# k-sheridan/mantis

Hardware: AMD Instinct MI355X
Metric: poses/sec + p50 per-frame latency, 1280x720 4-cam batch (higher is better)
Workload: dtype f64; 1 GPU; config3: 4-cam 1280x720 rig, shared map, full mantis3 path per camera + joint rig Gauss-Newton; cams_per_rig=4, contexts_per_gpu=6, landmarks=720, parallelism=rig-data-parallel x1

## Files before the change

### include/mantis.h

```cpp
#ifndef MANTIS_H
#define MANTIS_H
#include <stddef.h>
#include <stdint.h>

#ifdef __cplusplus
extern "C" {
#endif

#define MANTIS_ABI_VERSION 5

typedef enum mantis_status {
  MANTIS_OK = 0,
  MANTIS_ERR_ARG = 1,
  MANTIS_ERR_DEVICE = 2,
  MANTIS_ERR_OOM = 3,
  MANTIS_ERR_CAPACITY = 4,
  MANTIS_ERR_STATE = 5,
  MANTIS_ERR_COMM = 6
} mantis_status;

typedef enum mantis_reason {
  MANTIS_PUBLISHED = 0,
  MANTIS_NO_QUADS = 1,
  MANTIS_NO_HYPS = 2,
// ... 90 lines not shown
                                   mantis_result* out, mantis_cam_result* cam_out);

mantis_status mantis_process_rig_sharded(void* ctx, const mantis_image* local_cams, int32_t n_rigs, int32_t n_local,
                                         const int32_t* cam_index, int32_t cams_per_rig, mantis_result* out,
                                         mantis_cam_result* cam_out);

mantis_status mantis_shard_gauss_offsets(void* ctx, const int32_t* pairs, int32_t npairs, int32_t n_global,
                                         const int32_t* gidx, int32_t n_local, int32_t per_frame, int32_t* offsets,
                                         int32_t* total);

typedef struct mantis_rig_gn_info {
  double T_init[16];
  double T_final[16];
  double cost0, cost;
  int32_t valid, iterations, n_obs, n_obs_local;
} mantis_rig_gn_info;
mantis_status mantis_get_rig_gn(void* ctx, int32_t rig, mantis_rig_gn_info* info, double* obs, int32_t cap);

mantis_status mantis_get_rig_weights(void* ctx, int32_t rig, double* weights, double* c2w, double* sums,
                                     int32_t* chosen);
mantis_status mantis_get_rig_weights_info(void* ctx, int32_t* n_rigs, int32_t* cams_per_rig);

mantis_status mantis_markov_init(void* ctx, int32_t n_filters, const double* w2c_R);
mantis_status mantis_markov_sense(void* ctx, const double* w2c_R, const int32_t* active);
mantis_status mantis_markov_convolve(void* ctx, const double* dtheta, const double* dt, const int32_t* active);
mantis_status mantis_markov_weight(void* ctx, int32_t filter, const double* w2c_R, int32_t n, double* error);
mantis_status mantis_markov_get(void* ctx, double* planes, double* yaw, int32_t* argmax);

mantis_status mantis_canny(void* ctx, const mantis_image* img, uint8_t* canny_out);
mantis_status mantis_hysteresis(void* ctx, const uint8_t* cls, int32_t width, int32_t height, uint8_t* edges_out);
mantis_status mantis_masks(void* ctx, const mantis_image* img, uint8_t* det_out, uint8_t* mask_out);
mantis_status mantis_detect_quads(void* ctx, const mantis_image* img, int32_t* corners, int32_t max_quads,
                                  int32_t* n_quads);
mantis_status mantis_score_hypotheses(void* ctx, const mantis_image* img, const uint8_t* mask, const double* c2w,
                                      int32_t n, int32_t fast, double* err, int32_t* nproj);
mantis_status mantis_rpp_batch(void* ctx, const double* img_pts, const double* obj_pts, int32_t n, double* R,
                               double* t, double* errs, int32_t* rpp_status);
mantis_status mantis_rpp_solve(void* ctx, const double* img_pts, const double* obj_pts, int32_t n_points,
                               int32_t n, double* R, double* t, double* errs, int32_t* rpp_status,
                               int32_t* iterations);

mantis_status mantis_quad_gn(void* ctx, const double* img_pts, const double* obj_pts, int32_t n, double* R,
                             double* t, int32_t iterations, int32_t* steps, double* costs);

mantis_status mantis_score_argmin(void* ctx, const mantis_image* img, const uint8_t* mask, const double* c2w,
                                  int32_t n, int64_t index_base, int32_t use_comm, double* best_err,
                                  int64_t* best_idx);
mantis_status mantis_score_argmin_dev(void* ctx, const mantis_image* img, const uint8_t* mask_dev,
                                      const double* c2w_dev, int32_t n, int64_t index_base, int32_t use_comm,
                                      double* best_err, int64_t* best_idx);
mantis_status mantis_argmin_pick(const double* pairs, int32_t nranks, double* best_err, int64_t* best_idx);

mantis_status mantis_score_argmin_batch(void* ctx, const mantis_image* imgs, int32_t n_frames,
                                        const uint8_t* const* masks_dev, const double* const* c2w_dev,
                                        const int32_t* n_hyps, const int64_t* index_base, int32_t use_comm,
                                        double* best_err, int64_t* best_idx);

mantis_status mantis_gn_accumulate(void* ctx, const double* T_w_b, const double* T_base_cam, int32_t n_cams,
                                   const double* obs, int32_t n_obs, double* acc28);
mantis_status mantis_gn_solve(const double* acc28, double lambda, double* T_w_b, double* delta6);

mantis_status mantis_comm_unique_id(void* id128);
mantis_status mantis_comm_init(void* ctx, const void* id128, int32_t nranks, int32_t rank);
mantis_status mantis_comm_info(void* ctx, int32_t* nranks, int32_t* rank);
mantis_status mantis_gn_allreduce(void* ctx, double* acc28);

// ... 391 lines not shown
```

### mantis_amd/__init__.py

```python
import ctypes as C
import os

import numpy as np

ROOT = os.path.dirname(os.path.dirname(os.path.abspath(__file__)))
LIB_PATH = os.environ.get("MANTIS_AMD_LIB") or os.path.join(os.path.dirname(os.path.abspath(__file__)),
                                                             "libmantis_amd.so")

MANTIS_OK = 0
REASONS = {0: "published", 1: "no_quads", 2: "no_hyps", 3: "yaw_ambiguous", 4: "no_yaw"}


class MantisConfig(C.Structure):
    _fields_ = [("struct_size", C.c_int32), ("device", C.c_int32), ("max_cams", C.c_int32),
                ("max_width", C.c_int32), ("max_height", C.c_int32), ("rng_seed", C.c_uint64),
                ("canny_low", C.c_int32), ("polygon_epsilon", C.c_int32),
                ("search_radius_multiplier", C.c_double), ("grid_spacing", C.c_double),
                ("particles", C.c_int32), ("iterations", C.c_int32), ("gn_enable", C.c_int32),
                ("gn_iterations", C.c_int32), ("max_quads", C.c_int32), ("max_contour_points", C.c_int32),
                ("quad_gn_iterations", C.c_int32), ("rig_weighting", C.c_int32)]


class MantisImage(C.Structure):
    _fields_ = [("width", C.c_int32), ("height", C.c_int32), ("step_bytes", C.c_int32), ("mem_kind", C.c_int32),
# ... 191 lines not shown
        ("quads", (C.c_int32 * 8) * 256), ("test_pts", (C.c_double * 8) * 256),
        ("n_gen", C.c_int32), ("n_hyps", C.c_int32),
        ("hyp_c2w", (C.c_double * 12) * 1024), ("hyp_err", C.c_double * 1024), ("hyp_n", C.c_int32 * 1024),
        ("best1_c2w", C.c_double * 12), ("best1_err", C.c_double),
        ("pf_c2w", C.c_double * 12), ("pf_err", C.c_double), ("pf_iter_err", C.c_double * 11),
        ("shift_err", C.c_double * 81), ("top20_err", C.c_double * 20), ("yaw_err", C.c_double * 4),
        ("yaw_best", C.c_int32), ("min_yaw_diff", C.c_double), ("pub_c2w", C.c_double * 12),
        ("pub_error", C.c_double), ("position", C.c_double * 3), ("orientation_xyzw", C.c_double * 4),
        ("covariance", C.c_double * 36), ("rng_state_after", C.c_uint64), ("n_scored", C.c_int32),
    ]


_lib = None

_SIGS = {
    "mantis_abi_version": (C.c_int32, []),
    "mantis_default_config": (None, [C.POINTER(MantisConfig)]),
    "mantis_create": (C.c_int, [C.POINTER(MantisConfig), C.POINTER(C.c_void_p)]),
    "mantis_destroy": (C.c_int, [C.c_void_p]),
    "mantis_last_error": (C.c_char_p, [C.c_void_p]),
    "mantis_set_map": (C.c_int, [C.c_void_p, C.c_void_p, C.c_int32, C.c_void_p, C.c_int32, C.c_void_p, C.c_int32]),
    "mantis_parse_coordinates": (C.c_int32, [C.c_char_p, C.c_void_p, C.c_int32]),
    "mantis_rng_get": (C.c_int, [C.c_void_p, C.POINTER(C.c_uint64)]),
    "mantis_rng_set": (C.c_int, [C.c_void_p, C.c_uint64]),
    "mantis_process": (C.c_int, [C.c_void_p, C.POINTER(MantisImage), C.c_int32, C.POINTER(MantisMotion),
                                 C.POINTER(MantisResult), C.POINTER(MantisCamResult)]),
    "mantis_process_batch": (C.c_int, [C.c_void_p, C.POINTER(MantisImage), C.c_int32, C.c_int32,
                                       C.POINTER(MantisResult), C.POINTER(MantisCamResult)]),
    "mantis_canny": (C.c_int, [C.c_void_p, C.POINTER(MantisImage), C.c_void_p]),
    "mantis_hysteresis": (C.c_int, [C.c_void_p, C.c_void_p, C.c_int32, C.c_int32, C.c_void_p]),
    "mantis_masks": (C.c_int, [C.c_void_p, C.POINTER(MantisImage), C.c_void_p, C.c_void_p]),
    "mantis_detect_quads": (C.c_int, [C.c_void_p, C.POINTER(MantisImage), C.c_void_p, C.c_int32,
                                      C.POINTER(C.c_int32)]),
    "mantis_score_hypotheses": (C.c_int, [C.c_void_p, C.POINTER(MantisImage), C.c_void_p, C.c_void_p, C.c_int32,
                                          C.c_int32, C.c_void_p, C.c_void_p]),
    "mantis_rpp_batch": (C.c_int, [C.c_void_p, C.c_void_p, C.c_void_p, C.c_int32, C.c_void_p, C.c_void_p,
                                   C.c_void_p, C.c_void_p]),
    "mantis_small_batch_frames": (C.c_int32, [C.c_void_p]),
    "mantis_rpp_solve": (C.c_int, [C.c_void_p, C.c_void_p, C.c_void_p, C.c_int32, C.c_int32, C.c_void_p,
                                   C.c_void_p, C.c_void_p, C.c_void_p, C.c_void_p]),
    "mantis_quad_gn": (C.c_int, [C.c_void_p, C.c_void_p, C.c_void_p, C.c_int32, C.c_void_p, C.c_void_p, C.c_int32,
                                 C.c_void_p, C.c_void_p]),
    "mantis_get_rig_weights": (C.c_int, [C.c_void_p, C.c_int32, C.c_void_p, C.c_void_p, C.c_void_p,
                                         C.POINTER(C.c_int32)]),
    "mantis_markov_init": (C.c_int, [C.c_void_p, C.c_int32, C.c_void_p]),
    "mantis_markov_sense": (C.c_int, [C.c_void_p, C.c_void_p, C.c_void_p]),
    "mantis_markov_convolve": (C.c_int, [C.c_void_p, C.c_void_p, C.c_void_p, C.c_void_p]),
    "mantis_markov_weight": (C.c_int, [C.c_void_p, C.c_int32, C.c_void_p, C.c_int32, C.c_void_p]),
    "mantis_markov_get": (C.c_int, [C.c_void_p, C.c_void_p, C.c_void_p, C.c_void_p]),
    "mantis_set_prior_pose": (C.c_int, [C.c_void_p, C.c_void_p]),
    "mantis_get_prior_pose": (C.c_int, [C.c_void_p, C.c_void_p, C.POINTER(C.c_int32)]),
    "mantis_synth_render": (C.c_int, [C.c_void_p, C.POINTER(SynthCamC), C.c_int32, C.c_void_p, C.c_void_p]),
    "mantis_device_alloc": (C.c_int, [C.c_void_p, C.c_size_t, C.POINTER(C.c_void_p)]),
    "mantis_device_free": (C.c_int, [C.c_void_p, C.c_void_p]),
    "mantis_memcpy_h2d": (C.c_int, [C.c_void_p, C.c_void_p, C.c_void_p, C.c_size_t]),
    "mantis_memcpy_d2h": (C.c_int, [C.c_void_p, C.c_void_p, C.c_void_p, C.c_size_t]),
    "mantis_synchronize": (C.c_int, [C.c_void_p]),
    "mantis_kernel_times": (C.c_int32, [C.c_void_p, C.POINTER(C.c_char_p), C.POINTER(C.c_float), C.c_int32]),
    "mantis_set_profiling": (C.c_int, [C.c_void_p, C.c_int32]),
    "mantis_frame_debug_size": (C.c_size_t, []),
    "mantis_get_frame_debug": (C.c_int, [C.c_void_p, C.c_int32, C.c_void_p, C.c_size_t]),
    "mantis_get_contours": (C.c_int, [C.c_void_p, C.c_int32, C.c_void_p, C.c_void_p, C.c_int32, C.c_void_p, C.c_int32,
                                      C.c_void_p]),
    "mantis_frame_counters": (C.c_int32, [C.c_void_p, C.c_int32, C.c_void_p, C.c_int32]),
    "mantis_gn_accumulate": (C.c_int, [C.c_void_p, C.c_void_p, C.c_void_p, C.c_int32, C.c_void_p, C.c_int32,
                                       C.c_void_p]),
# ... 910 lines not shown
        return out[:k]

    def frame_debug(self, i):
        d = FrameDebug()
        assert C.sizeof(d) == lib().mantis_frame_debug_size(), "FrameDebug layout mismatch"
        self._chk(lib().mantis_get_frame_debug(self.h, i, C.byref(d), C.sizeof(d)), "get_frame_debug")
        return d

    def canny(self, img):
        out = np.zeros((img.height, img.width), np.uint8)
        self._chk(lib().mantis_canny(self.h, C.byref(img), out.ctypes.data), "canny")
        return out

    def hysteresis(self, cls):
        cls = np.ascontiguousarray(cls, np.uint8)
        h, w = cls.shape
        out = np.zeros((h, w), np.uint8)
        self._chk(lib().mantis_hysteresis(self.h, cls.ctypes.data, w, h, out.ctypes.data), "hysteresis")
        return out

    def masks(self, img):
        det = np.zeros((img.height, img.width), np.uint8)
        mask = np.zeros((img.height, img.width), np.uint8)
        self._chk(lib().mantis_masks(self.h, C.byref(img), det.ctypes.data, mask.ctypes.data), "masks")
        return det, mask

    def detect_quads(self, img, max_quads=256):
        corners = np.zeros((max_quads, 8), np.int32)
        n = C.c_int32()
        self._chk(lib().mantis_detect_quads(self.h, C.byref(img), corners.ctypes.data, max_quads, C.byref(n)),
                  "detect_quads")
        return corners[: n.value].copy()

    def score(self, img, c2w, fast=True, mask=None):
        c2w = np.ascontiguousarray(c2w, np.float64).reshape(-1, 12)
        n = len(c2w)
        err = np.zeros(n)
        npj = np.zeros(n, np.int32)
        mptr = None
        if mask is not None:
            mask = np.ascontiguousarray(mask, np.uint8)
            mptr = mask.ctypes.data
        self._chk(lib().mantis_score_hypotheses(self.h, C.byref(img), mptr, c2w.ctypes.data, n, int(fast),
                                                err.ctypes.data, npj.ctypes.data), "score_hypotheses")
        return err, npj

    def comm_init(self, rank, world, dist=None):
        uid = (C.c_uint8 * 128)()
        if rank == 0:
            self._chk(lib().mantis_comm_unique_id(uid), "comm_unique_id")
        if dist is not None and world > 1:
            box = [bytes(uid)]
            dist.broadcast_object_list(box, src=0)
            C.memmove(uid, box[0], 128)
        self._chk(lib().mantis_comm_init(self.h, uid, world, rank), "comm_init")

    def score_argmin(self, img, c2w, index_base=0, use_comm=False, mask=None):
        c2w = np.ascontiguousarray(c2w, np.float64).reshape(-1, 12)
        e = C.c_double()
        i = C.c_int64()
        mk = None if mask is None else np.ascontiguousarray(mask, np.uint8)
        self._chk(lib().mantis_score_argmin(self.h, C.byref(img), None if mk is None else mk.ctypes.data,
                                            c2w.ctypes.data, len(c2w), index_base, int(use_comm), C.byref(e),
                                            C.byref(i)), "score_argmin")
        return e.value, i.value

# ... 177 lines not shown
```

### mantis_amd/csrc/api.hip

```cpp
#include <hip/hip_runtime.h>
#ifndef MK_FC_THREADS
#define MK_FC_THREADS 256
#endif

#include <algorithm>
#include <atomic>
#include <cfloat>
#include <chrono>
#include <cmath>
#include <cstdio>
#include <cstdlib>
#include <cstring>
#include <mutex>
#include <sstream>
#include <string>
#include <thread>
#include <vector>

#include <rccl/rccl.h>

#include "hostbuf.h"
#include "kernels.hip"

namespace mk {
// ... 555 lines not shown
mantis_status run_hyst_ccl(Ctx* c, int n, int W, int H, bool edge_bytes) {
  const size_t P = c->plane, B = c->bstride;
  c->hyst_epoch = c->hyst_epoch >= 255 ? 4 : c->hyst_epoch + 1;
  if (c->hyst_epoch == 4) HIP_OK(hipMemsetAsync(c->d_strong, 0, c->fstride * (size_t)c->F, c->s));
  HystRuns hr{(uint32_t*)c->d_lroot.get(), c->d_lab, c->d_strong, c->d_rowb, c->lstride / 2, P, c->fstride, c->rstride, P / 2,
              HB_ROWS * ((W + 1) / 2), c->d_st, c->hyst_epoch};
  HIP_OK(hipMemset2DAsync(c->d_rowb + H + 1, c->rstride * sizeof(int32_t), 0, 2 * sizeof(int32_t), n, c->s));
  const int WWb = bits::words(W);
  k_hyst_band<<<dim3((H + HB_ROWS - 1) / HB_ROWS, n), HB_THREADS, 3 * sizeof(uint32_t) * HB_ROWS * WWb, c->s>>>(
      c->d_b1, c->d_b2, B, hr, c->d_eb, W, H);
  mark(c, "hysteresis/k_hyst_band");
  const int nseam = (H - 1) / HB_ROWS;
  if (nseam > 0) k_hyst_seam<<<dim3((nseam + 3) / 4, n), 256, 0, c->s>>>(hr, H);
  mark(c, "hysteresis/k_hyst_seam");
  k_hyst_mark<<<dim3(8, n), 256, 0, c->s>>>(hr, H);
  mark(c, "hysteresis/k_hyst_mark");
  k_hyst_fix<<<dim3(8, n), 256, 0, c->s>>>(hr, c->d_eb, B, W, H);
  if (edge_bytes) k_bits_to_bytes<<<blocks_for((size_t)W * H), 256, 0, c->s>>>(c->d_eb, c->d_edge, W, H, 0);
  mark(c, "hysteresis/k_hyst_fix");
  HIP_OK(hipGetLastError());
  return MANTIS_OK;
}

mantis_status run_contours(Ctx* c, int n, int W, int H) {
  const size_t P = c->plane;
  const int Wp = W + 2, Hp = H + 2;
  dim3 grow((Hp + 4 * RUN_RPW - 1) / (4 * RUN_RPW), n);
  uint16_t* rx = c->d_lroot;
  if (!c->runs_done) {
    k_run_count<<<grow, 256, 0, c->s>>>(c->d_dbits, c->dstride, c->d_rowb, c->rstride, Wp, Hp);
    k_run_scan<<<n, 256, 0, c->s>>>(c->d_rowb, c->rstride, c->d_st, Hp);
    k_run_emit<<<grow, 256, 0, c->s>>>(c->d_dbits, c->dstride, c->d_rowb, c->rstride, rx, c->d_lab, P, Wp, Hp);
  }
  k_run_band<<<dim3((Hp + RB_ROWS - 1) / RB_ROWS, n), RB_THREADS, 0, c->s>>>(c->d_rowb, c->rstride, rx, c->d_lab, P, Wp, Hp);
  const int seams = (Hp - 1) / RB_ROWS;
  if (seams > 0)
    k_run_seam<<<dim3((seams + 3) / 4, n), 256, 0, c->s>>>(c->d_rowb, c->rstride, rx, c->d_lab, P, Wp, Hp);
  k_run_border<<<grow, 256, 0, c->s>>>(c->d_rowb, c->rstride, rx, c->d_lab, P, c->d_borders, c->d_st, Wp, Hp,
                                       kMaxBorders);
  mark(c, "components");
  const size_t tb_lds = (size_t)dbits_wpw(Wp) * Hp * sizeof(uint32_t);
  k_seg_plan<<<n, 256, 0, c->s>>>(c->d_dbits, c->dstride, c->d_rowb, c->rstride, rx, c->d_lab, P, c->d_borders,
                                  c->d_st, c->d_scratch, c->pool_cap, Wp, Hp, kMaxBorders, c->seg_m);
  if (trace_on_lds(c, n, Wp, Hp)) {
    k_trace_borders_lds<<<n, 1024, tb_lds, c->s>>>(c->d_dbits, c->dstride, c->d_borders, c->d_st, c->d_scratch,
                                                   c->pool_cap, Wp, Hp, kMaxBorders, c->d_rowb, c->rstride, rx, P);
  } else {
    const int wpw = dbits_wpw(Wp);
    k_tile_bits<<<dim3((Hp + 31) / 32, n), 256, kTbRows * wpw * sizeof(uint32_t), c->s>>>(
        c->d_dbits, c->dstride, c->d_tbits, c->tstride, wpw, Wp, Hp);
    k_trace_borders<<<n, 64 * MK_TB_WAVES, 0, c->s>>>(c->d_tbits, c->tstride, c->d_borders, c->d_st, c->d_scratch, c->pool_cap, Wp,
                                        kMaxBorders, c->d_rowb, c->rstride, rx, P);
  }
  k_seg_chain<<<n, 256, 0, c->s>>>(c->d_st, c->d_bcount, c->d_scratch, c->pool_cap, kMaxBorders);
  mark(c, "border_trace");
  k_frame_contours<<<n, n <= c->fc_small_frames ? 1024 : MK_FC_THREADS, 0, c->s>>>(c->d_dbits, c->dstride, c->d_borders, c->d_st, c->d_bcount, c->d_boff,
                                         c->d_pool, c->d_scratch, c->pool_cap, c->d_quads, c->d_dbg, c->d_frames, Wp,
                                         Hp, P, kMaxBorders, (double)c->cfg.polygon_epsilon,
                                         c->cfg.search_radius_multiplier, c->d_rowb, c->rstride, rx);
  mark(c, "contours_quads");
  HIP_OK(hipGetLastError());
  return MANTIS_OK;
}

std::atomic<int> g_live_ctx[64];

unsigned objpose_blocks(const Ctx* c, size_t expected_jobs) {
  size_t b = (expected_jobs + 127) / 128;
  const int live = std::max(1, g_live_ctx[c->cfg.device & 63].load());
  const size_t cap = c->rpp_blocks > 0 ? (size_t)c->rpp_blocks : (size_t)std::max(64, 3 * c->n_cu / (2 * live));
  return (unsigned)std::max<size_t>(1, std::min(b, cap));
}
// ... 1147 lines not shown
    HIP_OK(hipMemcpyAsync(mask_out, c->d_mask, (size_t)W * H, hipMemcpyDeviceToHost, c->s));
  }
  HIP_OK(hipStreamSynchronize(c->s));
  for (size_t i = 0; det_out && i < (size_t)W * H; i++) det_out[i] = det_out[i] ? 255 : 0;
  for (size_t i = 0; mask_out && i < (size_t)W * H; i++) mask_out[i] = mask_out[i] ? 255 : 0;
  return MANTIS_OK;
}

mantis_status mantis_detect_quads(void* ctx, const mantis_image* img, int32_t* corners, int32_t max_quads,
                                  int32_t* n_quads) {
  Ctx* c = (Ctx*)ctx;
  if (c) bind_device(c);
  if (!c || !img || !n_quads) return MANTIS_ERR_ARG;
  int W, H;
  mantis_status st = stage_frames(c, img, 1, W, H);
  if (st != MANTIS_OK) return st;
  c->frame_rng.clear();
  if ((st = run_image_stages(c, 1, W, H)) != MANTIS_OK) return st;
  if ((st = run_contours(c, 1, W, H)) != MANTIS_OK) return st;
  HIP_OK(hipMemcpyAsync(c->h_st, c->d_st, sizeof(FrameState), hipMemcpyDeviceToHost, c->s));
  HIP_OK(hipStreamSynchronize(c->s));
  if (c->h_st[0].overflow) { c->err = "detect_quads: workspace capacity exceeded"; return MANTIS_ERR_CAPACITY; }
  int nq = c->h_st[0].n_quads;
  *n_quads = nq;
  if (corners && max_quads > 0) {
    std::vector<QuadRec> q(nq);
    HIP_OK(hipMemcpy(q.data(), c->d_quads, sizeof(QuadRec) * nq, hipMemcpyDeviceToHost));
    for (int i = 0; i < nq && i < max_quads; i++)
      for (int k = 0; k < 8; k++) corners[8 * i + k] = q[i].c[k];
  }
  return MANTIS_OK;
}

mantis_status mantis_score_hypotheses(void* ctx, const mantis_image* img, const uint8_t* mask, const double* c2w,
                                      int32_t n, int32_t fast, double* err, int32_t* nproj) {
  Ctx* c = (Ctx*)ctx;
  if (c) bind_device(c);
  if (!c || !img || !c2w || n <= 0 || !err || !nproj) return MANTIS_ERR_ARG;
  if (!c->d_lm) { c->err = "map not set"; return MANTIS_ERR_STATE; }
  int W, H;
  mantis_status st = stage_frames(c, img, 1, W, H);
  if (st != MANTIS_OK) return st;
  double* d_c2w = nullptr;
  double* d_err = nullptr;
  int32_t* d_np = nullptr;
  DevScratch ds(c);
  if (ds.get(&d_c2w, (size_t)12 * n) || ds.get(&d_err, (size_t)n) || ds.get(&d_np, (size_t)n)) return MANTIS_ERR_OOM;
  const uint8_t* d_mask = nullptr;
  if (mask) {
    HIP_OK(hipMemcpyAsync(c->d_mask, mask, (size_t)W * H, hipMemcpyHostToDevice, c->s));
    d_mask = c->d_mask;
  }
  HIP_OK(hipMemcpyAsync(d_c2w, c2w, sizeof(double) * 12 * n, hipMemcpyHostToDevice, c->s));
  Landmarks L = lmk_of(c);
  mark(c, "start");
  k_score_api<<<(n + kApiHyps - 1) / kApiHyps, 64 * kApiHyps, 0, c->s>>>(c->d_frames, d_mask, L, d_c2w, n, fast, d_err, d_np);
  mark(c, "score_api");
  HIP_OK(hipGetLastError());
  HIP_OK(hipMemcpyAsync(err, d_err, sizeof(double) * n, hipMemcpyDeviceToHost, c->s));
  HIP_OK(hipMemcpyAsync(nproj, d_np, sizeof(int32_t) * n, hipMemcpyDeviceToHost, c->s));
  HIP_OK(hipStreamSynchronize(c->s));
  finish_profile(c);
  return MANTIS_OK;
}

mantis_status mantis_quad_gn(void* ctx, const double* img_pts, const double* obj_pts, int32_t n, double* R,
// ... 202 lines not shown
```

### mantis_amd/csrc/kernels.hip

```cpp
#include <hip/hip_runtime.h>

#include <cfloat>
#include <cstdint>
#include <type_traits>

#include "mk_bits.h"
#include "mk_contour.h"
#include "mk_gn.h"
#include "mk_math.h"
#include "mk_rpp.h"
#include "mk_shard.h"
#include "mk_sort.h"
#include "mk_track.h"
#include "mk_types.h"
#include "synth.h"

namespace mk {

#ifndef MK_DPP_SCAN
#define MK_DPP_SCAN 1
#endif
__device__ inline int wave_incl_scan(int v, int lane) {
#if MK_DPP_SCAN
  (void)lane;
// ... 1707 lines not shown
        T &= T - 1;
        X[o] = (uint16_t)(32 * w + b);
        L[o] = o;
        o++;
      }
      base += __builtin_amdgcn_readlane(inc, 63);
    }
  }
}

__device__ inline int run_at(const uint16_t* x, int n, int v) {
  int lo = 0, hi = n - 1;
  while (lo < hi) {
    const int mid = (lo + hi + 1) >> 1;
    if ((int)x[mid] <= v) lo = mid;
    else hi = mid - 1;
  }
  return lo;
}

template <class UF>
__device__ inline void run_row_union(const uint16_t* X, int bp, int np, int by, int ny, int Wp, int lane,
                                     const UF& uni) {
  const uint16_t* Xp = X + bp;
  for (int j = lane; j < ny; j += 64) {
    const int fg = j & 1;
    const int a = X[by + j], b = (j + 1 < ny ? (int)X[by + j + 1] : Wp) - 1;
    const int lo = a - fg, hi = b + fg;
    for (int k = run_at(Xp, np, lo); k < np && (int)Xp[k] <= hi; k++)
      if ((k & 1) == fg) uni(by + j, bp + k);
  }
}

#ifndef MK_RB_ROWS
#define MK_RB_ROWS 32
#endif
constexpr int RB_ROWS = MK_RB_ROWS, RB_CAP = 128 * MK_RB_ROWS;
#ifndef MK_RB_THREADS
#define MK_RB_THREADS 512
#endif
constexpr int RB_THREADS = MK_RB_THREADS, RB_WAVES = RB_THREADS / 64;
__global__ __launch_bounds__(RB_THREADS) void k_run_band(const int32_t* __restrict__ rowb, size_t rstride,
                                                  const uint16_t* __restrict__ rx, int32_t* lab, size_t plane, int Wp,
                                                  int Hp) {
  __shared__ int32_t Ll[RB_CAP];
  __shared__ uint16_t Xl[RB_CAP];
  __shared__ int32_t rbl[RB_ROWS + 1];
  const int f = blockIdx.y, t = threadIdx.x, lane = t & 63, wave = t >> 6;
  const int y0 = blockIdx.x * RB_ROWS;
  if (y0 >= Hp) return;
  const int y1 = min(y0 + RB_ROWS, Hp);
  const int32_t* r = rowb + (size_t)f * rstride;
  const uint16_t* X = rx + (size_t)f * plane;
  int32_t* L = lab + (size_t)f * plane;
  const int g0 = r[y0], n = r[y1] - g0;
  if (n > RB_CAP) {
    const auto uni = [L](int a, int b) { uf_union_c(L, a, b); };
    for (int y = y0 + 1 + wave; y < y1; y += RB_WAVES) run_row_union(X, r[y - 1], r[y] - r[y - 1], r[y], r[y + 1] - r[y], Wp, lane, uni);
    return;
  }
  for (int i = t; i <= y1 - y0; i += RB_THREADS) rbl[i] = r[y0 + i] - g0;
  for (int i = t; i < n; i += RB_THREADS) {
    Xl[i] = X[g0 + i];
    Ll[i] = i;
  }
  __syncthreads();
  int* Li = Ll;
  const auto uni = [Li](int a, int b) { lds_union(Li, a, b); };
  for (int y = y0 + 1 + wave; y < y1; y += RB_WAVES) {
    const int q = y - y0;
    run_row_union(Xl, rbl[q - 1], rbl[q] - rbl[q - 1], rbl[q], rbl[q + 1] - rbl[q], Wp, lane, uni);
  }
  __syncthreads();
  for (int i = t; i < n; i += RB_THREADS) L[g0 + i] = g0 + lds_find(Ll, i);
}

__global__ __launch_bounds__(256) void k_run_seam(const int32_t* __restrict__ rowb, size_t rstride,
                                                  const uint16_t* __restrict__ rx, int32_t* lab, size_t plane, int Wp,
                                                  int Hp) {
  const int f = blockIdx.y;
  const int y = (blockIdx.x * 4 + (threadIdx.x >> 6) + 1) * RB_ROWS, lane = threadIdx.x & 63;
  if (y >= Hp) return;
  const int32_t* r = rowb + (size_t)f * rstride;
  int32_t* L = lab + (size_t)f * plane;
  const auto uni = [L](int a, int b) { uf_union_c(L, a, b); };
  run_row_union(rx + (size_t)f * plane, r[y - 1], r[y] - r[y - 1], r[y], r[y + 1] - r[y], Wp, lane, uni);
}

__device__ inline int run_at_row(const int32_t* rowb, int Hp, int id) {
  int lo = 0, hi = Hp - 1;
  while (lo < hi) {
    const int mid = (lo + hi + 1) >> 1;
    if (rowb[mid] <= id) lo = mid;
    else hi = mid - 1;
  }
  return lo;
}

__global__ __launch_bounds__(256) void k_run_border(const int32_t* __restrict__ rowb, size_t rstride,
                                                    const uint16_t* __restrict__ rx, int32_t* lab, size_t plane,
                                                    Border* __restrict__ borders, FrameState* st, int Wp, int Hp,
                                                    int cap) {
  const int f = blockIdx.y, lane = threadIdx.x & 63;
  const int ya = (blockIdx.x * 4 + (threadIdx.x >> 6)) * RUN_RPW, yb = min(ya + RUN_RPW, Hp);
  if (ya >= Hp) return;
  const int32_t* r = rowb + (size_t)f * rstride;
  const uint16_t* X = rx + (size_t)f * plane;
  int32_t* L = lab + (size_t)f * plane;
  const int nrow = yb - ya;
  const int rbq = lane <= nrow ? r[ya + lane] : 0x7fffffff;
  const int g0 = __builtin_amdgcn_readlane(rbq, 0), g1 = __builtin_amdgcn_readlane(rbq, nrow);
  const int nruns = r[Hp];
  const uint64_t below = (1ull << lane) - 1;
  for (int id = g0 + lane; __ballot(id < g1); id += 64) {
    const bool live = id < g1;
    int y = ya, by = g0;
#pragma unroll
    for (int k = 1; k < RUN_RPW; k++) {
      const int bk = __builtin_amdgcn_readlane(rbq, k);
      if (k < nrow && bk <= id) { y = ya + k; by = bk; }
    }
    const int j = id - by;
    const bool root = live && id != 0 && L[id] == id;
    Border b;
    if (root) {
      const int key = y * Wp + X[id];
      b.key = key;
      if (j & 1) {
        b.start = key; b.hole = 0; b.parent = key;
      } else {
        const int pr = uf_find_c(L, id - 1);
        b.start = key - 1; b.hole = 1; b.parent = -(pr + 1);
      }
    }
    const uint64_t m = __ballot(root);
    if (!m) continue;
    const int leader = __ffsll((unsigned long long)m) - 1;
    int base = 0;
    if (lane == leader) base = atomicAdd(&st[f].n_borders, __popcll(m));
    base = __builtin_amdgcn_readlane(base, leader);
    if (!root) continue;
    const int idx = base + __popcll(m & below);
    if (idx < cap) {
      borders[(size_t)f * cap + idx] = b;
      if (2 * (size_t)nruns <= plane) L[nruns + id] = idx;
    } else {
      atomicOr(&st[f].overflow, 1);
    }
  }
}

__device__ inline int fdx(int s) { return (int)((0x901Au >> (2 * s)) & 3u) - 1; }
__device__ inline int fdy(int s) { return (int)((0xA901u >> (2 * s)) & 3u) - 1; }

__device__ inline void build_next_lut(uint8_t* lut, int tid, int nthreads) {
  for (int e = tid; e < 512 * 8; e += nthreads) {
    const uint32_t p9 = (uint32_t)e >> 3;
    const int s = e & 7;
    const uint32_t m = nb8_from_rows(p9 & 7u, (p9 >> 3) & 7u, (p9 >> 6) & 7u);
    const uint32_t r = ((m | (m << 8)) >> (s + 1)) & 0xffu;
    lut[e] = r ? (uint8_t)((s + 1 + __builtin_ctz(r)) & 7) : (uint8_t)8;
  }
}

constexpr int kChunk = 16;
#ifndef MK_CHUNK_BUF
#define MK_CHUNK_BUF 2
#endif
struct ChunkEmit {
  int32_t* chunks;
  int32_t* owner;
  int32_t* ordv;
  int32_t* ccount;
  int32_t* counter;
  int max_chunks, border, cur, k, nch;
  bool ovf;
  int n_pts = 0;
#if MK_CHUNK_BUF
#if MK_CHUNK_BUF == 2
  uint32_t bp[8];
  __device__ uint32_t pk(int j) const { return bp[j]; }
// ... 320 lines not shown
      return false;
    }
  }
  w.first = 0;
  if (s != w.prev_s) {
    em(x - 1, y - 1);
    w.n++;
    w.prev_s = s;
  }
  const uint32_t np = w.pos + wdelta(s);
  if (np == w.spos && w.pos == w.p1) {
    nx = -1;
    return false;
  }
  w.pos = np;
  w.s = (s + 4) & 7;
  w.steps++;
  return true;
}

struct BitsRows {
  const uint32_t* b;
  int wpw;
  __device__ uint32_t row3(int x, int y) const {
    const uint32_t* p = b + (size_t)y * wpw + ((x - 1) >> 5);
    const uint64_t v = ((uint64_t)p[1] << 32) | p[0];
    return (uint32_t)(v >> ((x - 1) & 31)) & 7u;
  }
  __device__ uint32_t operator()(int x, int y) const { return nb8_from_rows(row3(x, y - 1), row3(x, y), row3(x, y + 1)); }
};
__global__ __launch_bounds__(256) void k_seg_plan(const uint32_t* __restrict__ dbits, size_t dstride,
                                                  const int32_t* __restrict__ rowb, size_t rstride,
                                                  const uint16_t* __restrict__ rx, int32_t* lab, size_t plane,
                                                  const Border* __restrict__ borders, FrameState* st,
                                                  int32_t* __restrict__ scratch, int pool_cap, int Wp, int Hp,
                                                  int border_cap, int M) {
  __shared__ int32_t rb[kSegRows + 1];
  __shared__ int32_t wsum[4];
  const int f = blockIdx.x, t = threadIdx.x, lane = t & 63, wave = t >> 6;
  const int32_t* r = rowb + (size_t)f * rstride;
  const uint16_t* X = rx + (size_t)f * plane;
  int32_t* L = lab + (size_t)f * plane;
  const int nruns = r[Hp];
  const int32_t* bidx = L + nruns;
  int nb = st[f].n_borders;
  if (nb > border_cap) nb = border_cap;
  SegTab T = seg_tab(scratch + 4 * (size_t)f * pool_cap, pool_cap);
  if (nb > T.cap) {
    if (t == 0) atomicOr(&st[f].overflow, 2);
    nb = T.cap;
  }
  const Border* bs = borders + (size_t)f * border_cap;
  const int nsr = M > 0 ? (Hp - 2) / M : 0;
  bool split = M > 0 && nsr > 0 && nsr <= kSegRows && 2 * (size_t)nruns <= plane;
  static_assert(kSegRows <= 512, "two passes of 256 sampled rows");
  int carry = 0;
  for (int pass = 0; pass < 2; pass++) {
    int v = 0;
    const int k = pass * 256 + t;
    if (split && k < nsr) {
      const int y = (k + 1) * M;
      v = 2 * ((r[y + 1] - r[y] - 1) >> 1);
    }
    const int inc = wave_incl_scan(v, lane);
    if (lane == 63) wsum[wave] = inc;
    __syncthreads();
    int o = carry;
    for (int q = 0; q < wave; q++) o += wsum[q];
    if (k < kSegRows) rb[k] = o + inc - v;
    carry += wsum[0] + wsum[1] + wsum[2] + wsum[3];
    __syncthreads();
  }
  int NC = split ? carry : 0;
  if (NC + nb > T.cap) {
    split = false;
    NC = 0;
  }
  if (t == 0) {
    st[f].seg_nc = NC;
    st[f].seg_m = split ? M : 0;
  }
  for (int k = t; k < nsr && split; k += 256) T.rowbase[k] = rb[k];
  const BitsRows nbh{dbits + (size_t)f * dstride, dbits_wpw(Wp)};
  if (split) {
    for (int k = 0; k < nsr; k++) {
// ... 178 lines not shown
      continue;
    }
    if (nidle == 64) {
      if (exhausted) break;
      continue;
    }
    int nx = -1;
    if (act && !walk_step(nbh.b, nbh.G, next_lut, em, w, M, r, X, T.rowbase, nx)) {
      act = false;
      finish(nx);
    }
  }
  if (lane == 0) atomicMax(&st[f].trace_ticks, (int32_t)(wall_clock64() - t_start));
}

extern __shared__ uint32_t tb_lds[];
struct BitsNBLds {
  int wpw;
  __device__ uint32_t row3(int x, int y) const {
    const int o = y * wpw + ((x - 1) >> 5);
    const uint64_t v = ((uint64_t)tb_lds[o + 1] << 32) | tb_lds[o];
    return (uint32_t)(v >> ((x - 1) & 31)) & 7u;
  }
  __device__ uint32_t operator()(int x, int y) const { return nb8_from_rows(row3(x, y - 1), row3(x, y), row3(x, y + 1)); }
};
template <class NB, class EM>
__device__ inline int walk_segment_lds(const NB& nb, const uint8_t* lut, EM& em, const Border& b, int Wp,
                                       uint32_t pos, int sd, int M, const int32_t* r, const uint16_t* X,
                                       const int32_t* rowbase, int& steps) {
  Walk w;
  if (sd == kSegStart) {
    if (!walk_start(nb, b.start % Wp, b.start / Wp, b.hole != 0, em, w)) {
      steps = 0;
      return -1;
    }
    w.first = 0;
  } else {
    seg_begin(nb, b, Wp, pos, sd, w);
  }
  for (;;) {
    const int x = (int)(w.pos & 0xffffu), y = (int)(w.pos >> 16);
    const uint32_t p9 = nb.row3(x, y - 1) | (nb.row3(x, y) << 3) | (nb.row3(x, y + 1) << 6);
    const int s = lut[(p9 << 3) | w.s];
    if (M > 0 && !w.first && y % M == 0) {
      const bool west = arc_has(w.s, s, 4);
      if (west || arc_has(w.s, s, 0)) {
        steps = w.steps;
        em.n_pts = w.n;
        return seg_id_at(x, y, west ? 0 : 1, M, r, X, rowbase);
      }
    }
    w.first = 0;
    if (s != w.prev_s) {
      em(x - 1, y - 1);
      w.n++;
      w.prev_s = s;
    }
    const uint32_t np = w.pos + wdelta(s);
    if (np == w.spos && w.pos == w.p1) break;
    w.pos = np;
    w.s = (s + 4) & 7;
    w.steps++;
  }
  steps = w.steps;
  em.n_pts = w.n;
  return -1;
// ... 2331 lines not shown
```

### mantis_amd/csrc/mk_types.h

```cpp
#pragma once
#include <cstdint>

#include "../../include/mantis.h"
#include "mk_math.h"
#include "mk_screen.h"

namespace mk {

constexpr int kLandmarksMax = 2048;
constexpr int kGaussPerFrame = 3000;
constexpr int kMaxQuads = 256;
constexpr int kMaxHyps = 4 * kMaxQuads;
constexpr int kMaxBorders = 8192;

struct FrameDesc {
  const uint8_t* bgr;
  int32_t w, h;
  Cam cam;
  ScreenCam scam;
};

struct Border {
  int32_t key;
  int32_t start;
// ... 46 lines not shown
  double top20_err[20];
  double yaw_err[4];
  int32_t yaw_best;
  double min_yaw_diff;
  double pub_c2w[12];
  double pub_error;
  double position[3];
  double orientation_xyzw[4];
  double covariance[36];
  uint64_t rng_state_after;
  int32_t n_scored;
};


struct FrameState {
  int32_t n_borders;
  int32_t n_points;
  int32_t n_raw_quads;
  int32_t n_quads;
  int32_t n_gen;
  int32_t n_hyps;
  int32_t reaches_pf;
  int32_t gauss_offset;
  int32_t overflow;
  int32_t n_runs;
  int32_t ticks[6];
  int32_t rpp_iters[2];
  int32_t trace_steps_max;
  int32_t n_chunks;
  int32_t trace_steps_sum;
  int32_t trace_ticks;
  int32_t seg_nc;
  int32_t seg_m;
};

struct GnCam {
  double R_cb[9];
  double t_cb[3];
};
struct RigGnIO {
  double Twb[16];
  double T0[16];
  double cost0, cost;
  int32_t valid, iterations, n_obs, done;
  int32_t n_obs_local, pad[3];
};
constexpr int kGnSlot = 32;

constexpr int kYawBins = 360;

struct MarkovOp {
  int32_t kind;
  int32_t bin;
  int32_t off;
  int32_t pad;
  double den;
  double E[181];
};


}
```

Measured before the change: 30580 rig poses/s.

## Fuse border emission into band union and segment planning via root candidate lists

Removes the separate k_run_border kernel, which scanned every run to find union-find roots. k_run_band now records root candidates, and for oversized bands every run as a candidate, into a per-frame scratch list. k_seg_plan then emits borders from that compact list, falling back to a full scan when the list overflows. This saves a kernel launch and a full pass over runs, but puts border emission on one block per frame and reuses scratch space that seg_plan also uses for its tables. It also adds a debug API for contours on binary planes and fixes n_pts on a failed walk start.

```diff
diff --git a/include/mantis.h b/include/mantis.h
--- a/include/mantis.h
+++ b/include/mantis.h
@@ -146,6 +146,7 @@
 mantis_status mantis_masks(void* ctx, const mantis_image* img, uint8_t* det_out, uint8_t* mask_out);
 mantis_status mantis_detect_quads(void* ctx, const mantis_image* img, int32_t* corners, int32_t max_quads,
                                   int32_t* n_quads);
+mantis_status mantis_contours_of_binary(void* ctx, const uint8_t* planes, int32_t n, int32_t width, int32_t height);
 mantis_status mantis_score_hypotheses(void* ctx, const mantis_image* img, const uint8_t* mask, const double* c2w,
                                       int32_t n, int32_t fast, double* err, int32_t* nproj);
 mantis_status mantis_rpp_batch(void* ctx, const double* img_pts, const double* obj_pts, int32_t n, double* R,
diff --git a/mantis_amd/__init__.py b/mantis_amd/__init__.py
--- a/mantis_amd/__init__.py
+++ b/mantis_amd/__init__.py
@@ -247,6 +247,7 @@
     "mantis_masks": (C.c_int, [C.c_void_p, C.POINTER(MantisImage), C.c_void_p, C.c_void_p]),
     "mantis_detect_quads": (C.c_int, [C.c_void_p, C.POINTER(MantisImage), C.c_void_p, C.c_int32,
                                       C.POINTER(C.c_int32)]),
+    "mantis_contours_of_binary": (C.c_int, [C.c_void_p, C.c_void_p, C.c_int32, C.c_int32, C.c_int32]),
     "mantis_score_hypotheses": (C.c_int, [C.c_void_p, C.POINTER(MantisImage), C.c_void_p, C.c_void_p, C.c_int32,
                                           C.c_int32, C.c_void_p, C.c_void_p]),
     "mantis_rpp_batch": (C.c_int, [C.c_void_p, C.c_void_p, C.c_void_p, C.c_int32, C.c_void_p, C.c_void_p,
@@ -1223,6 +1224,13 @@
                   "detect_quads")
         return corners[: n.value].copy()
 
+    def contours_of_binary(self, planes):
+        planes = np.ascontiguousarray(planes, np.uint8)
+        if planes.ndim == 2:
+            planes = planes[None]
+        n, h, w = planes.shape
+        self._chk(lib().mantis_contours_of_binary(self.h, planes.ctypes.data, n, w, h), "contours_of_binary")
+
     def score(self, img, c2w, fast=True, mask=None):
         c2w = np.ascontiguousarray(c2w, np.float64).reshape(-1, 12)
         n = len(c2w)
diff --git a/mantis_amd/csrc/api.hip b/mantis_amd/csrc/api.hip
--- a/mantis_amd/csrc/api.hip
+++ b/mantis_amd/csrc/api.hip
@@ -611,12 +611,11 @@
     k_run_scan<<<n, 256, 0, c->s>>>(c->d_rowb, c->rstride, c->d_st, Hp);
     k_run_emit<<<grow, 256, 0, c->s>>>(c->d_dbits, c->dstride, c->d_rowb, c->rstride, rx, c->d_lab, P, Wp, Hp);
   }
-  k_run_band<<<dim3((Hp + RB_ROWS - 1) / RB_ROWS, n), RB_THREADS, 0, c->s>>>(c->d_rowb, c->rstride, rx, c->d_lab, P, Wp, Hp);
+  k_run_band<<<dim3((Hp + RB_ROWS - 1) / RB_ROWS, n), RB_THREADS, 0, c->s>>>(c->d_rowb, c->rstride, rx, c->d_lab, P, Wp, Hp,
+                                                                             c->d_st, c->d_scratch, c->pool_cap);
   const int seams = (Hp - 1) / RB_ROWS;
   if (seams > 0)
     k_run_seam<<<dim3((seams + 3) / 4, n), 256, 0, c->s>>>(c->d_rowb, c->rstride, rx, c->d_lab, P, Wp, Hp);
-  k_run_border<<<grow, 256, 0, c->s>>>(c->d_rowb, c->rstride, rx, c->d_lab, P, c->d_borders, c->d_st, Wp, Hp,
-                                       kMaxBorders);
   mark(c, "components");
   const size_t tb_lds = (size_t)dbits_wpw(Wp) * Hp * sizeof(uint32_t);
   k_seg_plan<<<n, 256, 0, c->s>>>(c->d_dbits, c->dstride, c->d_rowb, c->rstride, rx, c->d_lab, P, c->d_borders,
@@ -1830,6 +1829,38 @@
   return MANTIS_OK;
 }
 
+mantis_status mantis_contours_of_binary(void* ctx, const uint8_t* planes, int32_t n, int32_t width, int32_t height) {
+  Ctx* c = (Ctx*)ctx;
+  if (c) bind_device(c);
+  if (!c || !planes) return MANTIS_ERR_ARG;
+  const int W = width, H = height;
+  if (n <= 0 || n > c->F) { c->err = "frame count exceeds max_cams"; return MANTIS_ERR_ARG; }
+  if (W <= 2 || H <= 2 || W > c->Wmax || H > c->Hmax) { c->err = "image size outside [3, max]"; return MANTIS_ERR_ARG; }
+  const int Wp = W + 2, Hp = H + 2, wpw = dbits_wpw(Wp);
+  std::vector<uint32_t> bits((size_t)wpw * Hp);
+  for (int f = 0; f < n; f++) {
+    std::fill(bits.begin(), bits.end(), 0u);
+    const uint8_t* pl = planes + (size_t)f * W * H;
+    for (int y = 0; y < H; y++)
+      for (int x = 0; x < W; x++)
+        if (pl[(size_t)y * W + x]) bits[(size_t)(y + 1) * wpw + ((x + 1) >> 5)] |= 1u << ((x + 1) & 31);
+    HIP_OK(hipMemcpy(c->d_dbits + (size_t)f * c->dstride, bits.data(), sizeof(uint32_t) * bits.size(), hipMemcpyHostToDevice));
+    FrameDesc& fd = c->h_frames[f];
+    std::memset(&fd, 0, sizeof(fd));
+    fd.w = W;
+    fd.h = H;
+    fd.cam.fx = fd.cam.fy = 1.0;
+  }
+  HIP_OK(hipMemcpyAsync(c->d_frames, c->h_frames, sizeof(FrameDesc) * n, hipMemcpyHostToDevice, c->s));
+  c->frame_rng.clear();
+  HIP_OK(hipMemsetAsync(c->d_st, 0, sizeof(FrameState) * n, c->s));
+  c->runs_done = false;
+  if (mantis_status st = run_contours(c, n, W, H); st != MANTIS_OK) return st;
+  HIP_OK(hipMemcpyAsync(c->h_st, c->d_st, sizeof(FrameState) * n, hipMemcpyDeviceToHost, c->s));
+  HIP_OK(hipStreamSynchronize(c->s));
+  return MANTIS_OK;
+}
+
 mantis_status mantis_score_hypotheses(void* ctx, const mantis_image* img, const uint8_t* mask, const double* c2w,
                                       int32_t n, int32_t fast, double* err, int32_t* nproj) {
   Ctx* c = (Ctx*)ctx;
diff --git a/mantis_amd/csrc/kernels.hip b/mantis_amd/csrc/kernels.hip
--- a/mantis_amd/csrc/kernels.hip
+++ b/mantis_amd/csrc/kernels.hip
@@ -1763,6 +1763,13 @@
   }
 }
 
+struct RootCands {
+  int2* e;
+  int cap;
+};
+__device__ inline RootCands root_cands(int32_t* scratch, int f, int pool_cap) {
+  return RootCands{(int2*)(scratch + 4 * (size_t)f * pool_cap), pool_cap};
+}
 #ifndef MK_RB_ROWS
 #define MK_RB_ROWS 32
 #endif
@@ -1773,10 +1780,12 @@
 constexpr int RB_THREADS = MK_RB_THREADS, RB_WAVES = RB_THREADS / 64;
 __global__ __launch_bounds__(RB_THREADS) void k_run_band(const int32_t* __restrict__ rowb, size_t rstride,
                                                   const uint16_t* __restrict__ rx, int32_t* lab, size_t plane, int Wp,
-                                                  int Hp) {
+                                                  int Hp, FrameState* st, int32_t* __restrict__ scratch,
+                                                  int pool_cap) {
   __shared__ int32_t Ll[RB_CAP];
   __shared__ uint16_t Xl[RB_CAP];
   __shared__ int32_t rbl[RB_ROWS + 1];
+  __shared__ int32_t ncand, cbase;
   const int f = blockIdx.y, t = threadIdx.x, lane = t & 63, wave = t >> 6;
   const int y0 = blockIdx.x * RB_ROWS;
   if (y0 >= Hp) return;
@@ -1784,12 +1793,21 @@
   const int32_t* r = rowb + (size_t)f * rstride;
   const uint16_t* X = rx + (size_t)f * plane;
   int32_t* L = lab + (size_t)f * plane;
+  const RootCands C = root_cands(scratch, f, pool_cap);
   const int g0 = r[y0], n = r[y1] - g0;
   if (n > RB_CAP) {
+    if (t == 0) cbase = atomicAdd(&st[f].n_cand, n);
     const auto uni = [L](int a, int b) { uf_union_c(L, a, b); };
     for (int y = y0 + 1 + wave; y < y1; y += RB_WAVES) run_row_union(X, r[y - 1], r[y] - r[y - 1], r[y], r[y + 1] - r[y], Wp, lane, uni);
+    __syncthreads();
+    for (int y = y0 + wave; y < y1; y += RB_WAVES)
+      for (int j = r[y] + lane; j < r[y + 1]; j += 64) {
+        const int pos = cbase + (j - g0);
+        if (pos < C.cap) C.e[pos] = make_int2(j, y);
+      }
     return;
   }
+  if (t == 0) ncand = 0;
   for (int i = t; i <= y1 - y0; i += RB_THREADS) rbl[i] = r[y0 + i] - g0;
   for (int i = t; i < n; i += RB_THREADS) {
     Xl[i] = X[g0 + i];
@@ -1803,7 +1821,35 @@
     run_row_union(Xl, rbl[q - 1], rbl[q] - rbl[q - 1], rbl[q], rbl[q + 1] - rbl[q], Wp, lane, uni);
   }
   __syncthreads();
-  for (int i = t; i < n; i += RB_THREADS) L[g0 + i] = g0 + lds_find(Ll, i);
+  const uint64_t below = (1ull << lane) - 1;
+  for (int i0 = 0; i0 < n; i0 += RB_THREADS) {
+    const int i = i0 + t;
+    bool root = false;
+    if (i < n) {
+      const int rt = lds_find(Ll, i);
+      L[g0 + i] = g0 + rt;
+      root = rt == i && g0 + i != 0;
+    }
+    const uint64_t m = __ballot(root);
+    if (!m) continue;
+    const int leader = __ffsll((unsigned long long)m) - 1;
+    int base = 0;
+    if (lane == leader) base = atomicAdd(&ncand, __popcll(m));
+    base = __builtin_amdgcn_readlane(base, leader);
+    if (root) Xl[base + __popcll(m & below)] = (uint16_t)i;
+  }
+  __syncthreads();
+  const int nc = ncand;
+  if (t == 0) cbase = atomicAdd(&st[f].n_cand, nc);
+  __syncthreads();
+  for (int k = t; k < nc; k += RB_THREADS) {
+    const int i = Xl[k], pos = cbase + k;
+    int q = 0;
+    static_assert(RB_ROWS <= 64, "row search steps 32 .. 1");
+    for (int s = 32; s > 0; s >>= 1)
+      if (q + s < y1 - y0 && rbl[q + s] <= i) q += s;
+    if (pos < C.cap) C.e[pos] = make_int2(g0 + i, y0 + q);
+  }
 }
 
 __global__ __launch_bounds__(256) void k_run_seam(const int32_t* __restrict__ rowb, size_t rstride,
@@ -1828,56 +1874,42 @@
   return lo;
 }
 
-__global__ __launch_bounds__(256) void k_run_border(const int32_t* __restrict__ rowb, size_t rstride,
-                                                    const uint16_t* __restrict__ rx, int32_t* lab, size_t plane,
-                                                    Border* __restrict__ borders, FrameState* st, int Wp, int Hp,
-                                                    int cap) {
-  const int f = blockIdx.y, lane = threadIdx.x & 63;
-  const int ya = (blockIdx.x * 4 + (threadIdx.x >> 6)) * RUN_RPW, yb = min(ya + RUN_RPW, Hp);
-  if (ya >= Hp) return;
-  const int32_t* r = rowb + (size_t)f * rstride;
-  const uint16_t* X = rx + (size_t)f * plane;
-  int32_t* L = lab + (size_t)f * plane;
-  const int nrow = yb - ya;
-  const int rbq = lane <= nrow ? r[ya + lane] : 0x7fffffff;
-  const int g0 = __builtin_amdgcn_readlane(rbq, 0), g1 = __builtin_amdgcn_readlane(rbq, nrow);
-  const int nruns = r[Hp];
-  const uint64_t below = (1ull << lane) - 1;
-  for (int id = g0 + lane; __ballot(id < g1); id += 64) {
-    const bool live = id < g1;
-    int y = ya, by = g0;
-#pragma unroll
-    for (int k = 1; k < RUN_RPW; k++) {
-      const int bk = __builtin_amdgcn_readlane(rbq, k);
-      if (k < nrow && bk <= id) { y = ya + k; by = bk; }
-    }
-    const int j = id - by;
-    const bool root = live && id != 0 && L[id] == id;
-    Border b;
-    if (root) {
-      const int key = y * Wp + X[id];
-      b.key = key;
-      if (j & 1) {
-        b.start = key; b.hole = 0; b.parent = key;
-      } else {
-        const int pr = uf_find_c(L, id - 1);
-        b.start = key - 1; b.hole = 1; b.parent = -(pr + 1);
-      }
-    }
-    const uint64_t m = __ballot(root);
-    if (!m) continue;
-    const int leader = __ffsll((unsigned long long)m) - 1;
-    int base = 0;
-    if (lane == leader) base = atomicAdd(&st[f].n_borders, __popcll(m));
-    base = __builtin_amdgcn_readlane(base, leader);
-    if (!root) continue;
-    const int idx = base + __popcll(m & below);
-    if (idx < cap) {
-      borders[(size_t)f * cap + idx] = b;
-      if (2 * (size_t)nruns <= plane) L[nruns + id] = idx;
+struct RunPlanes {
+  const int32_t* r;
+  const uint16_t* X;
+  int32_t* L;
+  int nruns;
+  bool map_fits;
+};
+__device__ inline void run_border_trip(const RunPlanes& P, bool live, int id, int y, Border* borders, int cap,
+                                       int32_t* nbord, int32_t* overflow, int Wp, int lane) {
+  int32_t* L = P.L;
+  const bool root = live && id != 0 && L[id] == id;
+  Border b;
+  if (root) {
+    const int j = id - P.r[y];
+    const int key = y * Wp + P.X[id];
+    b.key = key;
+    if (j & 1) {
+      b.start = key; b.hole = 0; b.parent = key;
     } else {
-      atomicOr(&st[f].overflow, 1);
-    }
+      const int pr = uf_find_c(L, id - 1);
+      b.start = key - 1; b.hole = 1; b.parent = -(pr + 1);
+    }
+  }
+  const uint64_t m = __ballot(root);
+  if (!m) return;
+  const int leader = __ffsll((unsigned long long)m) - 1;
+  int base = 0;
+  if (lane == leader) base = atomicAdd(nbord, __popcll(m));
+  base = __builtin_amdgcn_readlane(base, leader);
+  if (!root) return;
+  const int idx = base + __popcll(m & ((1ull << lane) - 1));
+  if (idx < cap) {
+    borders[idx] = b;
+    if (P.map_fits) L[P.nruns + id] = idx;
+  } else {
+    atomicOr(overflow, 1);
   }
 }
 
@@ -2264,25 +2296,49 @@
 __global__ __launch_bounds__(256) void k_seg_plan(const uint32_t* __restrict__ dbits, size_t dstride,
                                                   const int32_t* __restrict__ rowb, size_t rstride,
                                                   const uint16_t* __restrict__ rx, int32_t* lab, size_t plane,
-                                                  const Border* __restrict__ borders, FrameState* st,
+                                                  Border* borders, FrameState* st,
                                                   int32_t* __restrict__ scratch, int pool_cap, int Wp, int Hp,
                                                   int border_cap, int M) {
   __shared__ int32_t rb[kSegRows + 1];
   __shared__ int32_t wsum[4];
+  __shared__ int32_t nbord;
   const int f = blockIdx.x, t = threadIdx.x, lane = t & 63, wave = t >> 6;
   const int32_t* r = rowb + (size_t)f * rstride;
   const uint16_t* X = rx + (size_t)f * plane;
   int32_t* L = lab + (size_t)f * plane;
   const int nruns = r[Hp];
   const int32_t* bidx = L + nruns;
-  int nb = st[f].n_borders;
+  Border* bs = borders + (size_t)f * border_cap;
+  {
+    if (t == 0) nbord = 0;
+    __syncthreads();
+    const RunPlanes P{r, X, L, nruns, 2 * (size_t)nruns <= plane};
+    const RootCands C = root_cands(scratch, f, pool_cap);
+    const int nc = st[f].n_cand;
+    if (nc <= C.cap) {
+      for (int k0 = 0; k0 < nc; k0 += 256) {
+        const bool live = k0 + t < nc;
+        const int2 e = live ? C.e[k0 + t] : make_int2(0, 0);
+        run_border_trip(P, live, e.x, e.y, bs, border_cap, &nbord, &st[f].overflow, Wp, lane);
+      }
+    } else {
+      for (int i0 = 1; i0 < nruns; i0 += 256) {
+        const int id = i0 + t;
+        const bool live = id < nruns && L[id] == id;
+        run_border_trip(P, live, id, live ? run_at_row(r, Hp, id) : 0, bs, border_cap, &nbord, &st[f].overflow, Wp,
+                        lane);
+      }
+    }
+    __syncthreads();
+    if (t == 0) st[f].n_borders = nbord;
+  }
+  int nb = nbord;
   if (nb > border_cap) nb = border_cap;
   SegTab T = seg_tab(scratch + 4 * (size_t)f * pool_cap, pool_cap);
   if (nb > T.cap) {
     if (t == 0) atomicOr(&st[f].overflow, 2);
     nb = T.cap;
   }
-  const Border* bs = borders + (size_t)f * border_cap;
   const int nsr = M > 0 ? (Hp - 2) / M : 0;
   bool split = M > 0 && nsr > 0 && nsr <= kSegRows && 2 * (size_t)nruns <= plane;
   static_assert(kSegRows <= 512, "two passes of 256 sampled rows");
@@ -2527,6 +2583,7 @@
   if (sd == kSegStart) {
     if (!walk_start(nb, b.start % Wp, b.start / Wp, b.hole != 0, em, w)) {
       steps = 0;
+      em.n_pts = w.n;
       return -1;
     }
     w.first = 0;
diff --git a/mantis_amd/csrc/mk_types.h b/mantis_amd/csrc/mk_types.h
--- a/mantis_amd/csrc/mk_types.h
+++ b/mantis_amd/csrc/mk_types.h
@@ -102,6 +102,7 @@
   int32_t trace_ticks;
   int32_t seg_nc;
   int32_t seg_m;
+  int32_t n_cand;
 };
 
 struct GnCam {
```

New measurement: 31130 rig poses/s, median of 4. Within noise of the previous version (+1.8%).
